# huang-yh/GaussianFormer

Hardware: AMD Instinct MI355X
Metric: Gaussians/sec splatted into 200×200×16×18 voxel grid (fwd) (higher is better)
Workload: dtype f32

## Files before the change

gaussianformer_amd/csrc/splat_fwd.hip:

```cpp
#include <algorithm>

#include "gf_common.hpp"

#ifndef GF_TIMELINE
#define GF_TIMELINE 0
#endif

namespace gf {

struct PrepArgs {
    const float *means3D;
    const int *means_int;
    const float *opacity;
    const float *semantics;
    const int *radii;
    const float *cov3D;
    const int *points_int;
    const float *pts;
    float *records;
    uint2 *boxes;
    unsigned long long *bitmask;
    uint32_t *verify_flags;
    int P, N, H, W, D, nwords, nrow, nsx, nsy, per_axis, variant, nprep_blocks, verify, prescale, exact_det, lattice;
    uint32_t *tile_counters;
// ... 1849 lines not shown
                        int cn[3], in_[3], tt[3];
#pragma unroll
                        for (int q = 0; q < 3; ++q) {
                            bb[q] = s_db[64 * q + lane];
                            ii[q] = s_dw[64 * q + lane];
                        }
                        asm volatile("" : "+v"(bb[0]), "+v"(bb[1]), "+v"(bb[2]), "+v"(ii[0]), "+v"(ii[1]), "+v"(ii[2]));
#pragma unroll
                        for (int q = 0; q < 3; ++q) {
                            bb[q] = 64 * q + lane < nd ? bb[q] : 0ull;
                            ii[q] *= 64u;
                            cn[q] = __builtin_popcountll(bb[q]);
                        }
#pragma unroll
                        for (int q = 0; q < 3; ++q) in_[q] = wave_inclusive_scan(cn[q]);
#pragma unroll
                        for (int q = 0; q < 3; ++q) tt[q] = __builtin_amdgcn_readlane(in_[q], 63);
                        tot = tt[0] + tt[1] + tt[2];
                        if (tot <= kWList) {
                            extract(bb[0], ii[0], in_[0] - cn[0]);
                            extract(bb[1], ii[1], tt[0] + in_[1] - cn[1]);
                            extract(bb[2], ii[2], tt[0] + tt[1] + in_[2] - cn[2]);
                        } else {
                            fits = false;
                        }
                    } else {
                        for (int d0 = 0; d0 < nd; d0 += 64) {
                            const int i = d0 + lane;
                            const unsigned long long bits = i < nd ? s_db[i] : 0ull;
                            const uint32_t id0 = (i < nd ? s_dw[i] : 0u) * 64u;
                            const int cnt = __builtin_popcountll(bits);
                            const int incl = wave_inclusive_scan(cnt);
                            const int t = __builtin_amdgcn_readlane(incl, 63);
                            if (tot + t > kWList) {
                                fits = false;
                                break;
                            }
                            extract(bits, id0, tot + incl - cnt);
                            tot += t;
                        }
                    }
                    if (fits) {
                        list_len = tot;
                        c = nchunk;
                    }
                }
            }
            while (true) {
                bool last = false;
                if (LONG) {
                    uint32_t *d_lo = s_u, *d_hi = s_u + kLDense;
                    unsigned short *d_w = reinterpret_cast<unsigned short *>(s_u + 2 * kLDense);
                    if (!long_first) {
                        lds_dma16((gptr)(a.summary + (size_t)s * a.sum_pitch + 16 * min(lane, (a.sum_pitch >> 4) - 1)), (lptr)s_sum);
                        asm volatile("s_waitcnt vmcnt(0)" ::: "memory");
                    }
                    long_first = false;
                    const uint4 sv = reinterpret_cast<const uint4 *>(s_sum)[lane];
                    auto nib16 = [](uint32_t d) -> uint32_t {
                        uint32_t x = d & 0x0F0F0F0Fu;
                        x = (x | (x >> 4)) & 0x00FF00FFu;
                        return (x | (x >> 8)) & 0x0000FFFFu;
                    };
                    unsigned long long sm = (unsigned long long)(nib16(sv.x) | (nib16(sv.y) << 16)) |
                                            ((unsigned long long)(nib16(sv.z) | (nib16(sv.w) << 16)) << 32);
                    {
                        const int left = a.nwords - 64 * lane;
                        sm = left >= 64 ? sm : (left > 0 ? sm & bits_below(left) : 0ull);
                    }
                    const int cw = __builtin_popcountll(sm);
                    const int incl_w = wave_inclusive_scan(cw);
                    const int nd = __builtin_amdgcn_readlane(incl_w, 63);
                    const int cnt = min(nd - long_lo, kLDense);
                    {
                        unsigned long long m = sm;
                        int t = incl_w - cw - long_lo;
                        while (m) {
                            const int b = __builtin_ctzll(m);
                            m &= m - 1;
                            if ((unsigned)t < (unsigned)cnt) d_w[t] = (unsigned short)(64 * lane + b);
                            ++t;
                        }
                    }
                    __builtin_amdgcn_fence(__ATOMIC_ACQ_REL, "wavefront");
                    __builtin_amdgcn_wave_barrier();
                    const uint32_t *bm32 = reinterpret_cast<const uint32_t *>(bm);
                    for (int k0 = 0; k0 < cnt; k0 += 64) {
                        const uint32_t w = d_w[min(k0 + lane, cnt - 1)];
                        lds_dma4((gptr)(bm32 + 2 * w), (lptr)(d_lo + k0));
                        lds_dma4((gptr)(bm32 + 2 * w + 1), (lptr)(d_hi + k0));
                    }
                    asm volatile("s_waitcnt vmcnt(0)" ::: "memory");
                    int tot = 0, used = 0;
                    for (int k0 = 0; k0 < cnt; k0 += 64) {
                        const int j = k0 + lane;
                        const bool in = j < cnt;
                        const int jc = min(j, cnt - 1);
                        unsigned long long bits = (unsigned long long)d_lo[jc] | ((unsigned long long)d_hi[jc] << 32);
                        bits = in ? bits : 0ull;
                        const uint32_t id0 = (uint32_t)d_w[jc] * 64u;
                        const int cb = __builtin_popcountll(bits);
                        const int incl = wave_inclusive_scan(cb);
                        const int total = __builtin_amdgcn_readlane(incl, 63);
                        int pos = -1, adm = 64;
                        if (tot + total <= kLIds) {
                            pos = tot + incl - cb;
                        } else {
                            adm = 0;
                            int e_adm = 0;
                            for (int g8 = 0; g8 < 8; ++g8) {
                                const int e1 = __builtin_amdgcn_readlane(incl, 8 * g8 + 7);
                                if (tot + e1 > kLIds) break;
                                adm = 8 * (g8 + 1);
                                e_adm = e1;
                            }
                            if (lane < adm) pos = tot + incl - cb;
                            (void)e_adm;
                        }
                        if (pos >= 0) {
                            while (bits) {
                                const int b = __builtin_ctzll(bits);
                                bits &= bits - 1;
                                s_lg[pos++] = id0 + (uint32_t)b;
                            }
                        }
                        if (adm == 64) {
                            tot += total;
                            used += min(64, cnt - k0);
                        } else {
                            tot += adm ? __builtin_amdgcn_readlane(incl, max(adm - 1, 0)) : 0;
                            used += min(adm, cnt - k0);
                            break;
                        }
                    }
                    list_len = tot;
                    last = long_lo + used >= nd;
                    long_lo += used;
                }
                while (!LONG) {
                    if (c >= nchunk) {
                        last = true;
                        break;
                    }
                    const int w = 64 * c + lane;
                    unsigned long long bits = w < a.nwords ? s_row[w] : 0ull;
                    const int cnt = __builtin_popcountll(bits);
                    const int incl = wave_inclusive_scan(cnt);
                    const int total = __builtin_amdgcn_readlane(incl, 63);
                    int pos = -1;
                    if (total <= kWList) {
                        if (list_len + total > kWList) break;
                        pos = list_len + incl - cnt;
                        list_len += total;
                        ++c;
                    } else {
                        bool full = false;
                        for (; sg < 8; ++sg) {
                            const int e1 = __builtin_amdgcn_readlane(incl, 8 * sg + 7);
                            const int e0 = sg ? __builtin_amdgcn_readlane(incl, 8 * sg - 1) : 0;
                            if (list_len + (e1 - e0) > kWList) {
                                full = true;
                                break;
                            }
                            if ((lane >> 3) == sg) pos = list_len + (incl - cnt) - e0;
                            list_len += e1 - e0;
                        }
                        if (!full) {
                            sg = 0;
                            ++c;
                        }
                        if (pos >= 0) {
                            const uint32_t id0 = (uint32_t)w * 64u;
                            while (bits) {
                                const int j = __builtin_ctzll(bits);
                                bits &= bits - 1;
                                s_lg[pos++] = id0 + (uint32_t)j;
                            }
                        }
                        if (full) break;
                        continue;
                    }
                    const uint32_t id0 = (uint32_t)w * 64u;
                    while (bits) {
                        const int j = __builtin_ctzll(bits);
                        bits &= bits - 1;
                        s_lg[pos++] = id0 + (uint32_t)j;
                    }
                }
                __builtin_amdgcn_fence(__ATOMIC_ACQ_REL, "wavefront");
                __builtin_amdgcn_wave_barrier();
#if GF_TIMELINE
                if (!tl[2]) tl[2] = wall_clock64();
#endif
                for (int b0 = 0; b0 < list_len; b0 += 64) {
                    const uint32_t id = s_lg[min(b0 + lane, list_len - 1)];
                    lds_dma4((gptr)(&a.boxes[id].x), (lptr)(s_blo + b0));
                    lds_dma4((gptr)(&a.boxes[id].y), (lptr)(s_bhi + b0));
                }
                asm volatile("s_waitcnt vmcnt(0)" ::: "memory");
                if (PREP && a.rows_valid && r == 0 && !published) {
                    published = true;
                    constexpr int kPub = LONG ? kBwdPubLong : kBwdList;
                    if (last && list_len <= kPub) {
                        uint32_t *dst = a.pub_lists + (size_t)s * (3 * kPub);
                        for (int i = lane; i < list_len; i += 64) {
                            dst[i] = s_lg[i]; dst[kPub + i] = s_blo[i]; dst[2 * kPub + i] = s_bhi[i];
                        }
                        if (lane == 0) a.pub_len[s] = (uint32_t)list_len;
                    } else if (lane == 0) {
                        if (LONG) a.pub_len[s] = 0xFFFFFFFFu;
                        else atomicOr(const_cast<uint32_t *>(a.verify_flags) + (kListsBad - 64), 1u);
                    }
                }
#if GF_TIMELINE
                if (!tl[3]) tl[3] = wall_clock64();
#endif
                const int nbase = list_len + ((LONG && !last) ? 64 : 0);
                for (int base = 0; base < nbase || (last && base == 0); base += 64) {
                    const int i = base + lane;
                    const int ic = min(i, max(list_len - 1, 0));
                    const uint32_t eg = s_lg[ic];
                    const uint32_t blo = s_blo[ic], bhi = s_bhi[ic];
                    const bool hit = i < list_len && ux(blo) < Xw + 4 && ux(bhi) > Xw && uy(blo) < Y0 + 4 && uy(bhi) > Y0 &&
                                     uz(blo) < Zw + 8 && uz(bhi) > Zw;
                    const unsigned long long todo = __builtin_amdgcn_ballot_w64(hit);
                    if (hit) q_id[(qhead + qlen + (int)mbcnt(todo)) & (kQCap - 1)] = eg;
                    qlen += __builtin_popcountll(todo);
                    const bool final_batch = last && base + 64 >= list_len;
                    const bool flush = LONG && !last && base >= list_len;
                    while (true) {
                        if (npend == 0) {
                            if (!(qlen >= 32 || (final_batch && qlen > 0))) break;
                            npend = min(qlen, 32);
                            __builtin_amdgcn_fence(__ATOMIC_ACQ_REL, "wavefront");
                            __builtin_amdgcn_wave_barrier();
                            request_records_at(qhead, 0, npend);
                        }
                        const int avail = qlen - npend;
                        if (!(avail >= 32 || final_batch || flush)) break;
                        const int qn = npend;
                        asm volatile("s_waitcnt vmcnt(0)" ::: "memory");
#if GF_TIMELINE
                        if (!tl[4]) tl[4] = wall_clock64();
                        tl[7] += 1;
#endif
                        const bool live = n < qn;
                        const float4 r0 = slot[lane], r1 = slot[64 + lane], r2 = slot[128 + lane];
                        const float4 e0 = slot[192 + lane], e1 = slot[256 + lane], e2 = slot[320 + lane];
                        __builtin_amdgcn_fence(__ATOMIC_ACQ_REL, "wavefront");
                        __builtin_amdgcn_wave_barrier();
                        const int nnext = (flush && avail < 32) ? 0 : min(avail, 32);
                        if (nnext > 0) request_records_at(qhead, qn, nnext);
                        const bool last_group = final_batch && nnext == 0;
                        if (last_group && lane == 0)
                            asm volatile("global_atomic_add %0, %1, %2, off sc0" : "=v"(claimed) : "v"(ctr), "v"(1u) : "memory");
                        {
                            const float opa = live ? r0.w : 0.f;
                            const float v[10] = {e0.x, e0.y, e0.z, e0.w, e1.x, e1.y, e1.z, e1.w, e2.x, e2.y};
#pragma unroll
                            for (int k = 0; k < 10; ++k) S[(8 * h + k) * kSRow + n] = opa * v[k];
                        }
                        H8 t1, t2, t3;
                        {
                            const double L = 1.4426950408889634074;
                            const double c0 = r1.x, c1 = r1.y, c2 = r1.z, c3 = r1.w, c4 = r2.x, c5 = r2.y;
                            double th[5];
                            if (h == 0) {
                                const double ex = Cx - (double)r0.x, ey = Cy - (double)r0.y, ez = Cz - (double)r0.z;
                                const double gx = c0 * ex + c3 * ey + c5 * ez, gy = c3 * ex + c1 * ey + c4 * ez, gz = c5 * ex + c4 * ey + c2 * ez;
                                th[0] = -0.5 * L * (ex * gx + ey * gy + ez * gz);
                                th[1] = -L * sx * gx; th[2] = -L * sy * gy; th[3] = -L * sz * gz;
                                th[4] = -0.5 * L * sx * sx * c0;
                            } else {
                                th[0] = -0.5 * L * sy * sy * c1; th[1] = -0.5 * L * sz * sz * c2;
                                th[2] = -L * sx * sy * c3; th[3] = -L * sy * sz * c4; th[4] = -L * sx * sz * c5;
                            }
#pragma unroll
                            for (int j = 0; j < 5; ++j) split3(live ? th[j] : 0.0, t1.e[j], t2.e[j], t3.e[j]);
#pragma unroll
                            for (int j = 5; j < 8; ++j) { t1.e[j] = (_Float16)0.f; t2.e[j] = (_Float16)0.f; t3.e[j] = (_Float16)0.f; }
                        }
                        H8 tb;
                        {
                            const uint32_t glo = __float_as_uint(r2.z), ghi = __float_as_uint(r2.w);
                            const int x0 = ux(glo) - Xw, x1 = ux(ghi) - Xw, y0 = uy(glo) - Y0, y1 = uy(ghi) - Y0;
                            const int z0 = uz(glo) - Zw, z1 = uz(ghi) - Zw;
                            typedef short i16x2 __attribute__((ext_vector_type(2)));
                            auto dup = [](int v) { return i16x2{(short)v, (short)v}; };
                            const i16x2 lo_a = dup(h ? z0 : x0), hi_a = dup((h ? z1 : x1) - 1);
                            const i16x2 lo_b = dup(h ? z0 : y0), hi_b = dup((h ? z1 : y1) - 1);
                            const short j4 = h ? 4 : 0;
                            const i16x2 dead = dup(live ? 0 : -1);
#pragma unroll
                            for (int k = 0; k < 4; ++k) {
                                const short j0 = (short)(2 * (k & 1)) + (k < 2 ? (short)0 : j4);
                                const i16x2 jj = i16x2{j0, (short)(j0 + 1)};
                                const i16x2 out = ((jj - (k < 2 ? lo_a : lo_b)) | ((k < 2 ? hi_a : hi_b) - jj) | dead) >> (short)15;
                                tb.u[k] = __builtin_bit_cast(uint32_t, out) & 0xF800F800u;
                            }
                        }
                        __builtin_amdgcn_fence(__ATOMIC_ACQ_REL, "wavefront");
                        __builtin_amdgcn_wave_barrier();
                        H8 sh[2], sl[2];
#pragma unroll
                        for (int q = 0; q < 4; ++q) {
                            const float4 v4 = *reinterpret_cast<const float4 *>(S + min(n, kC) * kSRow + 8 * q + 4 * h);
                            const fp16x2 ha = __builtin_amdgcn_cvt_pkrtz(v4.x, v4.y), hb = __builtin_amdgcn_cvt_pkrtz(v4.z, v4.w);
                            float ra0, ra1, rb0, rb1;
                            asm("v_fma_mix_f32 %0, %1, -1.0, %2 op_sel_hi:[1,0,0]" : "=v"(ra0) : "v"(ha), "v"(v4.x));
                            asm("v_fma_mix_f32 %0, %1, -1.0, %2 op_sel:[1,0,0] op_sel_hi:[1,0,0]" : "=v"(ra1) : "v"(ha), "v"(v4.y));
                            asm("v_fma_mix_f32 %0, %1, -1.0, %2 op_sel_hi:[1,0,0]" : "=v"(rb0) : "v"(hb), "v"(v4.z));
                            asm("v_fma_mix_f32 %0, %1, -1.0, %2 op_sel:[1,0,0] op_sel_hi:[1,0,0]" : "=v"(rb1) : "v"(hb), "v"(v4.w));
                            sh[q >> 1].p[2 * (q & 1)] = ha; sh[q >> 1].p[2 * (q & 1) + 1] = hb;
                            sl[q >> 1].p[2 * (q & 1)] = __builtin_amdgcn_cvt_pkrtz(ra0, ra1); sl[q >> 1].p[2 * (q & 1) + 1] = __builtin_amdgcn_cvt_pkrtz(rb0, rb1);
                        }
                        auto pair = [&](int b0) {
                            f32x16 d0, d1;
#pragma unroll
                            for (int q = 0; q < 16; ++q) { d0[q] = 0.f; d1[q] = 0.f; }
                            d0 = __builtin_amdgcn_mfma_f32_32x32x16_f16(t3.v, phi[b0], d0, 0, 0, 0);
                            d1 = __builtin_amdgcn_mfma_f32_32x32x16_f16(t3.v, phi[b0 + 1], d1, 0, 0, 0);
                            d0 = __builtin_amdgcn_mfma_f32_32x32x16_f16(t2.v, phi[b0], d0, 0, 0, 0);
                            d1 = __builtin_amdgcn_mfma_f32_32x32x16_f16(t2.v, phi[b0 + 1], d1, 0, 0, 0);
                            d0 = __builtin_amdgcn_mfma_f32_32x32x16_f16(t1.v, phi[b0], d0, 0, 0, 0);
                            d1 = __builtin_amdgcn_mfma_f32_32x32x16_f16(t1.v, phi[b0 + 1], d1, 0, 0, 0);
                            d0 = __builtin_amdgcn_mfma_f32_32x32x16_f16(tb.v, hot[b0], d0, 0, 0, 0);
                            d1 = __builtin_amdgcn_mfma_f32_32x32x16_f16(tb.v, hot[b0 + 1], d1, 0, 0, 0);
                            H8 wh[2][2], wl[2][2];
                            auto weights = [&](const f32x16 &d, int k) {
#pragma unroll
                                for (int q = 0; q < 16; q += 2) {
                                    const float w0 = __builtin_amdgcn_exp2f(d[q]), w1 = __builtin_amdgcn_exp2f(d[q + 1]);
                                    const fp16x2 hi = __builtin_amdgcn_cvt_pkrtz(w0, w1);
                                    float q0, q1;
                                    asm("v_fma_mix_f32 %0, %1, -1.0, %2 op_sel_hi:[1,0,0]" : "=v"(q0) : "v"(hi), "v"(w0));
                                    asm("v_fma_mix_f32 %0, %1, -1.0, %2 op_sel:[1,0,0] op_sel_hi:[1,0,0]" : "=v"(q1) : "v"(hi), "v"(w1));
                                    wh[k][q >> 3].p[(q & 7) >> 1] = hi;
                                    wl[k][q >> 3].p[(q & 7) >> 1] = __builtin_amdgcn_cvt_pkrtz(q0, q1);
                                }
                            };
                            weights(d0, 0);
                            weights(d1, 1);
#pragma unroll
                            for (int kh = 0; kh < 2; ++kh) {
#pragma unroll
                                for (int k = 0; k < 2; ++k) acc[b0 + k] = __builtin_amdgcn_mfma_f32_32x32x16_f16(sl[kh].v, wh[k][kh].v, acc[b0 + k], 0, 0, 0);
#pragma unroll
                                for (int k = 0; k < 2; ++k) acc[b0 + k] = __builtin_amdgcn_mfma_f32_32x32x16_f16(sh[kh].v, wl[k][kh].v, acc[b0 + k], 0, 0, 0);
#pragma unroll
                                for (int k = 0; k < 2; ++k) acc[b0 + k] = __builtin_amdgcn_mfma_f32_32x32x16_f16(sh[kh].v, wh[k][kh].v, acc[b0 + k], 0, 0, 0);
                            }
                        };
                        pair(0);
                        pair(2);
                        have_next = have_next || last_group;
                        qhead = (qhead + qn) & (kQCap - 1);
                        qlen -= qn;
                        npend = nnext;
                    }
                }
                if (last) break;
                list_len = 0;
            }
#if GF_TIMELINE
            asm volatile("" :: "v"(acc[0]), "v"(acc[1]), "v"(acc[2]), "v"(acc[3]));
            tl[5] = wall_clock64();
#endif
            if (!have_next && lane == 0)
                asm volatile("global_atomic_add %0, %1, %2, off sc0" : "=v"(claimed) : "v"(ctr), "v"(1u) : "memory");
            asm volatile("s_waitcnt vmcnt(0)" : "+v"(claimed)::"memory");
            have_next = true;
            {
                const int nl = __builtin_amdgcn_readfirstlane((int)claimed);
                const int q2 = (int)__umulhi((uint32_t)nl, m_ps);
                if (nl < per_xcd && 8 * q2 + xcd < a.nsx * a.nsy) {
                    const int s2 = 8 * q2 + xcd, r2 = nl - q2 * per_super;
                    const int srow2 = a.nsy == 1 ? s2 : (int)__umulhi((uint32_t)s2, m_nsy), scol2 = s2 - srow2 * a.nsy;
                    if (srow2 * kSuper + 4 * (r2 & 1) < a.H && scol2 * kSuper + 4 * ((r2 >> 1) & 1) < a.W) {
                        if (LONG) {
                            lds_dma16((gptr)(a.summary + (size_t)s2 * a.sum_pitch + 16 * min(lane, (a.sum_pitch >> 4) - 1)), (lptr)s_sum);
                        } else {
                            const unsigned long long *bm2 = a.bitmask + (size_t)s2 * a.nrow;
                            for (int i = 0; 128 * i < a.nrow; ++i)
                                if (128 * i + 2 * lane < a.nrow)
                                    lds_dma16((gptr)(bm2 + 128 * i + 2 * lane), (lptr)(s_row + 128 * i));
                        }
                        next_row = true;
                    }
                }
            }
            typedef __attribute__((address_space(1))) float gfloat;
            typedef float nt4v __attribute__((ext_vector_type(4), aligned(4)));
            typedef __attribute__((address_space(1))) nt4v nt4;
            if ((a.D & 3) == 0) {
#pragma unroll
                for (int b = 0; b < 4; ++b) {
                    float *row = stage + ((b >> 1) * 64 + 32 * (b & 1) + n) * kC;
                    *reinterpret_cast<float2 *>(row + 4 * h) = make_float2(acc[b][0], acc[b][1]);
                    *reinterpret_cast<float2 *>(row + 4 * h + 2) = make_float2(acc[b][2], acc[b][3]);
                    *reinterpret_cast<float2 *>(row + 8 + 4 * h) = make_float2(acc[b][4], acc[b][5]);
                    *reinterpret_cast<float2 *>(row + 10 + 4 * h) = make_float2(acc[b][6], acc[b][7]);
                    if (h == 0) *reinterpret_cast<float2 *>(row + 16) = make_float2(acc[b][8], acc[b][9]);
                }
                auto labels_from_stage = [&]() {
#pragma unroll
                    for (int half = 0; half < 2; ++half) {
                        const int l = lane;
                        const float *row = stage + (64 * half + l) * kC;
                        float best = row[0];
                        int arg = 0;
#pragma unroll
                        for (int ch = 1; ch < kC; ++ch) {
                            const float v = row[ch];
                            if (v > best) { best = v; arg = ch; }
                        }
                        const int cx = Xw + (l >> 4), cy = Y0 + ((l >> 2) & 3), cz = Zw + 4 * half + (l & 3);
                        if (cx < a.H && cy < a.W && cz < a.D) a.out_labels[((size_t)cx * a.W + cy) * a.D + cz] = arg;
                    }
                };
                if (LABELS) {
                    __builtin_amdgcn_fence(__ATOMIC_ACQ_REL, "wavefront");
                    __builtin_amdgcn_wave_barrier();
                    labels_from_stage();
                }
                if (!LABELS || a.out_logits) {
                uint32_t off[10];
                uint32_t okbits = 0u;
#pragma unroll
                for (int j = 0; j < 5; ++j) {
                    const int i = lane + 64 * j;
                    const int run = i / kC, k = i - run * kC;
                    const int cx = Xw + (run >> 2), cy = Y0 + (run & 3);
                    const bool okc = i < 16 * kC && cx < a.H && cy < a.W;
                    const uint32_t o = (uint32_t)((((size_t)cx * a.W + cy) * a.D + Zw) * kC + 4 * k);
#pragma unroll
                    for (int half = 0; half < 2; ++half) {
                        const bool ok = okc && Zw + 4 * half < a.D;
                        okbits |= ok ? (1u << (5 * half + j)) : 0u;
                        off[5 * half + j] = ok ? o + 4 * kC * half : 0u;
                    }
                }
                nst = ((!LABELS) && Xw + 4 <= a.H && Y0 + 4 <= a.W && Zw + 8 <= a.D) ? 10 : -1;
                asm volatile("" : "+v"(off[0]), "+v"(off[1]), "+v"(off[2]), "+v"(off[3]), "+v"(off[4]), "+v"(off[5]), "+v"(off[6]),
                             "+v"(off[7]), "+v"(off[8]), "+v"(off[9]));
                __builtin_amdgcn_fence(__ATOMIC_ACQ_REL, "wavefront");
                __builtin_amdgcn_wave_barrier();
                gfloat *obase = (gfloat *)a.out_logits;
                float4 val[10];
#pragma unroll
                for (int it = 0; it < 10; ++it)
                    val[it] = *reinterpret_cast<const float4 *>(stage + (it / 5) * 64 * kC + 4 * (lane + 64 * (it % 5)));
#pragma unroll
                for (int it = 0; it < 10; ++it) {
                    if (okbits & (1u << it))
                        __builtin_nontemporal_store((nt4v){val[it].x, val[it].y, val[it].z, val[it].w}, (nt4 *)(obase + off[it]));
                }
                }
            } else {
#pragma unroll
                for (int b = 0; b < 4; ++b) {
                    float *row = stage + ((b >> 1) * 64 + 32 * (b & 1) + n) * kC;
#pragma unroll
                    for (int q = 0; q < 10; ++q) {
                        const int ch = (q & 3) + 8 * (q >> 2) + 4 * h;
                        if (ch < kC) row[ch] = acc[b][q];
                    }
                }
                __builtin_amdgcn_fence(__ATOMIC_ACQ_REL, "wavefront");
                __builtin_amdgcn_wave_barrier();
                if (!LABELS || a.out_logits)
                    for (int i = lane; i < 2 * 64 * kC; i += 64) {
                        const int half = i / (64 * kC), l = (i % (64 * kC)) / kC, ch = i % kC;
                        const int cx = Xw + (l >> 4), cy = Y0 + ((l >> 2) & 3), cz = Zw + 4 * half + (l & 3);
                        if (cx < a.H && cy < a.W && cz < a.D) a.out_logits[(((size_t)cx * a.W + cy) * a.D + cz) * kC + ch] = stage[i];
                    }
                if (LABELS) {
#pragma unroll
                    for (int half = 0; half < 2; ++half) {
                        const int l = lane;
                        const float *row = stage + (64 * half + l) * kC;
                        float best = row[0];
                        int arg = 0;
                        for (int ch = 1; ch < kC; ++ch) {
                            const float v = row[ch];
                            if (v > best) { best = v; arg = ch; }
                        }
                        const int cx = Xw + (l >> 4), cy = Y0 + ((l >> 2) & 3), cz = Zw + 4 * half + (l & 3);
                        if (cx < a.H && cy < a.W && cz < a.D) a.out_labels[((size_t)cx * a.W + cy) * a.D + cz] = arg;
                    }
                }
            }
            asm volatile("s_waitcnt lgkmcnt(0)" ::: "memory");
#if GF_TIMELINE
            tl[6] = wall_clock64();
            if (a.timeline && lane == 0)
#pragma unroll
                for (int k = 0; k < 8; ++k) a.timeline[8 * (size_t)logical + k] = tl[k];
#endif
        }
        if (!have_next) {
            if (lane == 0) asm volatile("global_atomic_add %0, %1, %2, off sc0" : "=v"(claimed) : "v"(ctr), "v"(1u) : "memory");
            asm volatile("s_waitcnt vmcnt(0)" : "+v"(claimed)::"memory");
        }
        local = __builtin_amdgcn_readfirstlane((int)claimed);
        row_there = next_row;
        nst_prev = nst;
    }
}

static int mfma_wave_grid(int nunits)
{
    static int cus = 0;
    if (cus == 0) {
        int dev = 0, n = 0;
        if (hipGetDevice(&dev) != hipSuccess || hipDeviceGetAttribute(&n, hipDeviceAttributeMultiprocessorCount, dev) != hipSuccess || n <= 0) n = 256;
        cus = n;
    }
    const int per_xcd = (nunits + 7) / 8;
    return 8 * std::min(per_xcd, std::max(1, 8 * cus / 8));
}

struct BoxVolArgs {
    const int *means_int;
    const int *radii;
    uint32_t *tiles_touched;
    unsigned long long *num_rendered;
    int P, H, W, D, per_axis;
};

__global__ __launch_bounds__(256) void gf_box_volumes_kernel(BoxVolArgs a)
{
    const int g = blockIdx.x * 256 + threadIdx.x;
    uint32_t vol = 0;
    if (g < a.P) {
        int lo[3], hi[3];
        gaussian_box(a.means_int, a.radii, a.per_axis, g, a.H, a.W, a.D, lo, hi);
        vol = (uint32_t)(hi[2] - lo[2]) * (uint32_t)(hi[1] - lo[1]) * (uint32_t)(hi[0] - lo[0]);
        a.tiles_touched[g] = vol;
    }
    unsigned long long s = vol;
#pragma unroll
    for (int d = 32; d >= 1; d >>= 1) s += __shfl_xor(s, d, 64);
    if (lane_id() == 0 && s) atomicAdd(a.num_rendered, s);
}

static int mfma_grid(int ntiles_total)
{
    static int cus = 0;
    if (cus == 0) {
        int dev = 0, n = 0;
        if (hipGetDevice(&dev) != hipSuccess || hipDeviceGetAttribute(&n, hipDeviceAttributeMultiprocessorCount, dev) != hipSuccess || n <= 0) n = 256;
        cus = n;
    }
    const int per_xcd = (ntiles_total + 7) / 8;
    return 8 * std::min(per_xcd, std::max(1, 2 * cus / 8));
}

static int mfma_wave_units(int nsuper, int D) { return nsuper * 4 * ((D + 7) / 8); }

static bool mfma_by_wave(int nrow)
{
    return nrow <= kWRow && option(kOptSplatTileKernel) == 0;
}
static bool mfma_by_wave_long(int nrow, int nwords, int flags)
{
    return nrow > kWRow && nwords <= kLongWords && (flags & GF_WORKSPACE_ZEROED) && option(kOptSplatTileKernel) == 0;
}

static int mfma_kind(int nrow, int P, int flags = 0)
{
    return (mfma_by_wave(nrow) || mfma_by_wave_long(nrow, (P + 63) / 64, flags)) ? 1 : 0;
}

static uint32_t mfma_counter_init(int kind, int nsuper, int D)
{
    return kind == 1 ? (uint32_t)(mfma_wave_grid(mfma_wave_units(nsuper, D)) / 8) : (uint32_t)(mfma_grid(nsuper * kTilesPerSuper) / 8);
}

static void launch_render_mfma(const RenderArgs &r, int nsuper, hipStream_t stream)
{
    hipEvent_t ev0, ev1;
    const bool prof = profile_slot(&ev0, &ev1);
    if (prof) (void)hipEventRecord(ev0, stream);
    const int kind = mfma_kind(r.nrow, r.P, r.summary ? GF_WORKSPACE_ZEROED : 0);
    const int wave_grid = mfma_wave_grid(mfma_wave_units(nsuper, r.D));
    if (kind == 1 && r.nrow > kWRow && r.out_labels)
        hipLaunchKernelGGL((gf_splat_render_mfma_wave_kernel<true, false, true>), dim3(wave_grid), dim3(64), 0, stream, r);
    else if (kind == 1 && r.nrow > kWRow && r.rows_valid)
        hipLaunchKernelGGL((gf_splat_render_mfma_wave_kernel<false, true, true>), dim3(wave_grid), dim3(64), 0, stream, r);
    else if (kind == 1 && r.nrow > kWRow)
        hipLaunchKernelGGL((gf_splat_render_mfma_wave_kernel<false, false, true>), dim3(wave_grid), dim3(64), 0, stream, r);
    else if (kind == 1 && r.out_labels)
        hipLaunchKernelGGL(gf_splat_render_mfma_wave_kernel<true>, dim3(wave_grid), dim3(64), 0, stream, r);
    else if (kind == 1 && r.rows_valid)
        hipLaunchKernelGGL((gf_splat_render_mfma_wave_kernel<false, true>), dim3(wave_grid), dim3(64), 0, stream, r);
    else if (kind == 1)
        hipLaunchKernelGGL(gf_splat_render_mfma_wave_kernel<false>, dim3(wave_grid), dim3(64), 0, stream, r);
    else
        hipLaunchKernelGGL(gf_splat_render_mfma_kernel<false>, dim3(mfma_grid(r.ntiles_total)), dim3(kBlock), 0, stream, r);
    if (prof) (void)hipEventRecord(ev1, stream);
}

template <int VARIANT, int EXP, bool LABELS>
static void launch_render(bool dense_candidate, const RenderArgs &r, hipStream_t stream)
{
    if (dense_candidate) {
        const int per_xcd = ((r.nsx * r.nsy + 7) / 8) * kTilesPerSuper;
        hipEvent_t ev0, ev1;
        const bool prof = profile_slot(&ev0, &ev1);
        if (prof) (void)hipEventRecord(ev0, stream);
        hipLaunchKernelGGL((gf_splat_render_kernel<VARIANT, EXP, LABELS>), dim3(per_xcd * 8), dim3(kBlock), 0, stream, r);
        if (prof) (void)hipEventRecord(ev1, stream);
    } else {
        const int blocks = (int)min((long long)4096, ((long long)r.N + kBlock - 1) / kBlock);
        hipLaunchKernelGGL((gf_splat_render_general_kernel<VARIANT, EXP, LABELS>), dim3(blocks), dim3(kBlock), 0, stream, r);
    }
}

static int exp_flavour(int variant, int flags)
{
    if (flags & GF_LIBM_EXP) return kExpLibm;
    if (flags & GF_COMP_EXP) return kExpComp;
    if (flags & GF_FAST_EXP) return kExpFast;
    return variant == GF_SPLAT_PROB ? kExpComp : kExpFast;
}

template <int VARIANT>
static void launch_render_exp(int flags, bool dense_candidate, const RenderArgs &r, hipStream_t stream)
{
    const int ex = exp_flavour(VARIANT, flags);
    if (r.out_labels) {
        if (ex == kExpLibm) launch_render<VARIANT, kExpLibm, true>(dense_candidate, r, stream);
        else if (ex == kExpComp) launch_render<VARIANT, kExpComp, true>(dense_candidate, r, stream);
        else launch_render<VARIANT, kExpFast, true>(dense_candidate, r, stream);
        return;
    }
    if (ex == kExpLibm) launch_render<VARIANT, kExpLibm, false>(dense_candidate, r, stream);
    else if (ex == kExpComp) launch_render<VARIANT, kExpComp, false>(dense_candidate, r, stream);
    else launch_render<VARIANT, kExpFast, false>(dense_candidate, r, stream);
}

void launch_prep_for_backward(int radii_per_axis, int P, int N, int H, int W, int D, const float *pts, const int *points_int,
                              const float *means3D, const int *means3D_int, const float *opacity, const float *semantics,
                              const int *radii, const float *cov3D, const uint32_t *state, const SplatWorkspace &ws, hipStream_t stream)
{
    PrepArgs pa;
    pa.means3D = means3D; pa.means_int = means3D_int; pa.opacity = opacity; pa.semantics = semantics;
    pa.radii = radii; pa.cov3D = cov3D; pa.points_int = points_int; pa.pts = pts; pa.records = ws.records; pa.boxes = ws.boxes;
    pa.bitmask = ws.bitmask; pa.verify_flags = ws.flags + 64; pa.P = P; pa.N = N; pa.H = H; pa.W = W; pa.D = D;
    pa.nwords = ws.nwords; pa.nrow = ws.nrow; pa.nsx = ws.nsx; pa.nsy = ws.nsy; pa.per_axis = radii_per_axis ? 1 : 0;
    const int prep_waves = P >= 65536 ? 4 : 2;
    pa.variant = GF_SPLAT_BASE; pa.nprep_blocks = (ws.nwords + prep_waves - 1) / prep_waves; pa.verify = 0;
    pa.prescale = 0; pa.exact_det = 0; pa.lattice = 0;
    pa.tile_counters = nullptr; pa.tile_counter_init = 0u;
    pa.range_flags = nullptr; pa.range_theta_here = 0; pa.verdict_words = nullptr;
    pa.summary = nullptr; pa.sum_pitch = 0;
    pa.unit_totals = ws.bwd_wave_total; pa.unit_local = ws.bwd_row_local; pa.bwd_counters = ws.flags + kBwdCounters;
// ... 188 lines not shown
```

Before: 683.0 million.

## Software-pipeline MFMA exponent, exp2 weight split, and accumulate across four blocks

Restructures the inner splat step so the exponent MFMAs for the next block and the accumulate MFMAs for the previous block are interleaved with the exp2/fp16-split weight computation of the current block. Explicit sched_barriers pin the order. The goal is to hide MFMA latency behind VALU transcendental work. The pipelined path is enabled only for certain template configurations (LONG, or neither LABELS nor PREP). It keeps four d accumulators and four weight sets live at once, which raises register pressure.

```diff
diff --git a/gaussianformer_amd/csrc/splat_fwd.hip b/gaussianformer_amd/csrc/splat_fwd.hip
--- a/gaussianformer_amd/csrc/splat_fwd.hip
+++ b/gaussianformer_amd/csrc/splat_fwd.hip
@@ -2175,8 +2175,7 @@
                         __builtin_amdgcn_fence(__ATOMIC_ACQ_REL, "wavefront");
                         __builtin_amdgcn_wave_barrier();
                         H8 sh[2], sl[2];
-#pragma unroll
-                        for (int q = 0; q < 4; ++q) {
+                        auto s_split = [&](int q) {
                             const float4 v4 = *reinterpret_cast<const float4 *>(S + min(n, kC) * kSRow + 8 * q + 4 * h);
                             const fp16x2 ha = __builtin_amdgcn_cvt_pkrtz(v4.x, v4.y), hb = __builtin_amdgcn_cvt_pkrtz(v4.z, v4.w);
                             float ra0, ra1, rb0, rb1;
@@ -2186,46 +2185,66 @@
                             asm("v_fma_mix_f32 %0, %1, -1.0, %2 op_sel:[1,0,0] op_sel_hi:[1,0,0]" : "=v"(rb1) : "v"(hb), "v"(v4.w));
                             sh[q >> 1].p[2 * (q & 1)] = ha; sh[q >> 1].p[2 * (q & 1) + 1] = hb;
                             sl[q >> 1].p[2 * (q & 1)] = __builtin_amdgcn_cvt_pkrtz(ra0, ra1); sl[q >> 1].p[2 * (q & 1) + 1] = __builtin_amdgcn_cvt_pkrtz(rb0, rb1);
-                        }
-                        auto pair = [&](int b0) {
-                            f32x16 d0, d1;
-#pragma unroll
-                            for (int q = 0; q < 16; ++q) { d0[q] = 0.f; d1[q] = 0.f; }
-                            d0 = __builtin_amdgcn_mfma_f32_32x32x16_f16(t3.v, phi[b0], d0, 0, 0, 0);
-                            d1 = __builtin_amdgcn_mfma_f32_32x32x16_f16(t3.v, phi[b0 + 1], d1, 0, 0, 0);
-                            d0 = __builtin_amdgcn_mfma_f32_32x32x16_f16(t2.v, phi[b0], d0, 0, 0, 0);
-                            d1 = __builtin_amdgcn_mfma_f32_32x32x16_f16(t2.v, phi[b0 + 1], d1, 0, 0, 0);
-                            d0 = __builtin_amdgcn_mfma_f32_32x32x16_f16(t1.v, phi[b0], d0, 0, 0, 0);
-                            d1 = __builtin_amdgcn_mfma_f32_32x32x16_f16(t1.v, phi[b0 + 1], d1, 0, 0, 0);
-                            d0 = __builtin_amdgcn_mfma_f32_32x32x16_f16(tb.v, hot[b0], d0, 0, 0, 0);
-                            d1 = __builtin_amdgcn_mfma_f32_32x32x16_f16(tb.v, hot[b0 + 1], d1, 0, 0, 0);
-                            H8 wh[2][2], wl[2][2];
-                            auto weights = [&](const f32x16 &d, int k) {
-#pragma unroll
-                                for (int q = 0; q < 16; q += 2) {
-                                    const float w0 = __builtin_amdgcn_exp2f(d[q]), w1 = __builtin_amdgcn_exp2f(d[q + 1]);
-                                    const fp16x2 hi = __builtin_amdgcn_cvt_pkrtz(w0, w1);
-                                    float q0, q1;
-                                    asm("v_fma_mix_f32 %0, %1, -1.0, %2 op_sel_hi:[1,0,0]" : "=v"(q0) : "v"(hi), "v"(w0));
-                                    asm("v_fma_mix_f32 %0, %1, -1.0, %2 op_sel:[1,0,0] op_sel_hi:[1,0,0]" : "=v"(q1) : "v"(hi), "v"(w1));
-                                    wh[k][q >> 3].p[(q & 7) >> 1] = hi;
-                                    wl[k][q >> 3].p[(q & 7) >> 1] = __builtin_amdgcn_cvt_pkrtz(q0, q1);
+                        };
+                        f32x16 d[4];
+                        H8 wh[4][2], wl[4][2];
+                        auto expo = [&](int b, int j) {
+                            d[b] = __builtin_amdgcn_mfma_f32_32x32x16_f16(j == 0 ? t3.v : j == 1 ? t2.v : j == 2 ? t1.v : tb.v, j < 3 ? phi[b] : hot[b], d[b], 0, 0, 0);
+                        };
+                        auto weights = [&](int b, int c) {
+                            const int q = 2 * c;
+                            const float w0 = __builtin_amdgcn_exp2f(d[b][q]), w1 = __builtin_amdgcn_exp2f(d[b][q + 1]);
+                            const fp16x2 hi = __builtin_amdgcn_cvt_pkrtz(w0, w1);
+                            float q0, q1;
+                            asm("v_fma_mix_f32 %0, %1, -1.0, %2 op_sel_hi:[1,0,0]" : "=v"(q0) : "v"(hi), "v"(w0));
+                            asm("v_fma_mix_f32 %0, %1, -1.0, %2 op_sel:[1,0,0] op_sel_hi:[1,0,0]" : "=v"(q1) : "v"(hi), "v"(w1));
+                            wh[b][q >> 3].p[(q & 7) >> 1] = hi;
+                            wl[b][q >> 3].p[(q & 7) >> 1] = __builtin_amdgcn_cvt_pkrtz(q0, q1);
+                        };
+                        auto accum = [&](int b, int m) {
+                            const int kh = m / 3, term = m % 3;
+                            acc[b] = __builtin_amdgcn_mfma_f32_32x32x16_f16(term == 0 ? sl[kh].v : sh[kh].v, term == 1 ? wl[b][kh].v : wh[b][kh].v, acc[b], 0, 0, 0);
+                        };
+#pragma unroll
+                        for (int b = 0; b < 4; ++b)
+#pragma unroll
+                            for (int q = 0; q < 16; ++q) d[b][q] = 0.f;
+                        constexpr bool kPipeline = LONG || !(LABELS || PREP);
+                        if constexpr (!kPipeline) {
+#pragma unroll
+                            for (int q = 0; q < 4; ++q) s_split(q);
+#pragma unroll
+                            for (int b0 = 0; b0 < 4; b0 += 2) {
+#pragma unroll
+                                for (int j = 0; j < 4; ++j) { expo(b0, j); expo(b0 + 1, j); }
+#pragma unroll
+                                for (int c = 0; c < 8; ++c) weights(b0, c);
+#pragma unroll
+                                for (int c = 0; c < 8; ++c) weights(b0 + 1, c);
+#pragma unroll
+                                for (int m = 0; m < 6; ++m) { accum(b0, m); accum(b0 + 1, m); }
+                            }
+                        } else {
+#pragma unroll
+                            for (int q = 0; q < 4; ++q) {
+                                s_split(q);
+                                expo(0, q);
+                            }
+                            __builtin_amdgcn_sched_barrier(0);
+#pragma unroll
+                            for (int b = 0; b < 4; ++b) {
+#pragma unroll
+                                for (int c = 0; c < 8; ++c) {
+                                    weights(b, c);
+                                    if (c < 3 && b > 0) { accum(b - 1, 2 * c); accum(b - 1, 2 * c + 1); }
+                                    if (c >= 3 && c < 7 && b < 3) expo(b + 1, c - 3);
+                                    if (c >= 4 && c < 7 && b == 3) accum(3, c - 4);
+                                    __builtin_amdgcn_sched_barrier(0);
                                 }
-                            };
-                            weights(d0, 0);
-                            weights(d1, 1);
-#pragma unroll
-                            for (int kh = 0; kh < 2; ++kh) {
-#pragma unroll
-                                for (int k = 0; k < 2; ++k) acc[b0 + k] = __builtin_amdgcn_mfma_f32_32x32x16_f16(sl[kh].v, wh[k][kh].v, acc[b0 + k], 0, 0, 0);
-#pragma unroll
-                                for (int k = 0; k < 2; ++k) acc[b0 + k] = __builtin_amdgcn_mfma_f32_32x32x16_f16(sh[kh].v, wl[k][kh].v, acc[b0 + k], 0, 0, 0);
-#pragma unroll
-                                for (int k = 0; k < 2; ++k) acc[b0 + k] = __builtin_amdgcn_mfma_f32_32x32x16_f16(sh[kh].v, wh[k][kh].v, acc[b0 + k], 0, 0, 0);
                             }
-                        };
-                        pair(0);
-                        pair(2);
+#pragma unroll
+                            for (int m = 3; m < 6; ++m) accum(3, m);
+                        }
                         have_next = have_next || last_group;
                         qhead = (qhead + qn) & (kQCap - 1);
                         qlen -= qn;
```

Result: faster. 693.9 million, median of 6 (+1.6%).
